# lesliegaga/GPT-SoVITS

Hardware: AMD Instinct MI355X
Metric: synthesised audio sec/sec (1/RTF), v2 pipeline (higher is better)
Workload: dtype f16

## Files before the change

gpt-sovits_amd/csrc/attn.hip:

```cpp
#include <stdlib.h>

#include "engine.h"

#define GSV_PIN() do { asm volatile("" ::: "memory"); __builtin_amdgcn_sched_barrier(0); } while (0)

namespace gsv {

__device__ __forceinline__ f4 mma16(h8 a, h8 b, f4 c) { return __builtin_amdgcn_mfma_f32_16x16x32_f16(a, b, c, 0, 0, 0); }

__global__ __launch_bounds__(256) void vt_kernel(const _Float16* __restrict__ v, int ld, int T, int ldv, _Float16* __restrict__ vt,
                                                 int heads, _Float16* __restrict__ q, int ldq, _Float16* __restrict__ k, int ldk,
                                                 const float* __restrict__ rope_cs, int rope_half, int planes, long long xz,
                                                 long long vtz) {
  const int row = blockIdx.z / planes, plane = blockIdx.z - row * planes;
  v += row * xz; q += row * xz; k += row * xz; vt += row * vtz;
  if (plane == heads) {
    const int n = T * rope_half * 2;
    const int stride = gridDim.x * gridDim.y * 256;
    for (int i = (blockIdx.y * gridDim.x + blockIdx.x) * 256 + threadIdx.x; i < n; i += stride) {
      const int which = i / (T * rope_half);
      const int rr = i - which * T * rope_half;
      const int t = rr / rope_half, p = rr - t * rope_half;
      _Float16* x = (which ? k + (long long)t * ldk : q + (long long)t * ldq) + 2 * p;
      const float c = rope_cs[((long long)t * rope_half + p) * 2], sn = rope_cs[((long long)t * rope_half + p) * 2 + 1];
// ... 142 lines not shown
}

template <int QT>
static int launch_flash_qt(const void* q, int ldq, const void* k, int ldk, const void* vt_buf, int ldv, int T, int heads, float scale,
                           void* out, int ldo, hipStream_t s, int rows, long long xz, long long vtz, long long oz) {
  const size_t lds = ((size_t)4 * 16 * QT * 68 + 8 * 16 * QT) * 4;
  static bool attr = false;
  if (!attr) {
    GSV_HIP(hipFuncSetAttribute((const void*)flash_attn64_f16_kernel<QT>, hipFuncAttributeMaxDynamicSharedMemorySize, (int)lds));
    attr = true;
  }
  hipLaunchKernelGGL(flash_attn64_f16_kernel<QT>, dim3(cdiv(T, 16 * QT), rows * heads), dim3(256), lds, s, (const _Float16*)q, ldq,
                     (const _Float16*)k, ldk, (const _Float16*)vt_buf, ldv, T, scale, (_Float16*)out, ldo, heads, xz, vtz, oz);
  GSV_HIP(hipGetLastError());
  return GSV_OK;
}

__device__ __forceinline__ int4 seg_find(const int4* __restrict__ tab, int n_seg, int x, bool by_tile) {
  int lo = 0, hi = n_seg - 1;
  while (lo < hi) {
    const int mid = (lo + hi + 1) >> 1;
    const int4 e = tab[mid];
    if ((by_tile ? e.w : e.z) <= x) lo = mid; else hi = mid - 1;
  }
  return tab[lo];
}

__global__ __launch_bounds__(256) void vt_seg_kernel(const _Float16* __restrict__ v, int ld, const int4* __restrict__ tab, int n_seg,
                                                     int ldv, _Float16* __restrict__ vt) {
  __shared__ _Float16 tile[32][34];
  const int head = blockIdx.z, j0 = blockIdx.x * 32, c0 = blockIdx.y * 32;
  const int4 sg = seg_find(tab, n_seg, j0, false);
  const int k0 = j0 - sg.z;
  const int tx = threadIdx.x & 31, ty = threadIdx.x >> 5;
  for (int i = ty; i < 32; i += 8) {
    const int j = k0 + i;
    tile[i][tx] = j < sg.y ? v[(long long)(sg.x + j) * ld + head * 64 + c0 + tx] : (_Float16)0.f;
  }
  __syncthreads();
  for (int i = ty; i < 32; i += 8) vt[((long long)head * 64 + c0 + i) * ldv + j0 + tx] = tile[tx][i];
}

template <int QT>
__global__ __launch_bounds__(256) void flash_attn64_seg_f16_kernel(const _Float16* __restrict__ q, int ldq, const _Float16* __restrict__ k,
                                                                   int ldk, const _Float16* __restrict__ vt, int ldv,
                                                                   const int4* __restrict__ tab, int n_seg, float scale,
                                                                   _Float16* __restrict__ out, int ldo) {
  const int vid = xcd_virtual_id(blockIdx.y * gridDim.x + blockIdx.x, gridDim.x * gridDim.y);
  const int head = vid / gridDim.x, tile = vid % gridDim.x;
  const int4 sg = seg_find(tab, n_seg, tile, true);
  flash_attn64_tile<QT>(q + (long long)sg.x * ldq, ldq, k + (long long)sg.x * ldk, ldk, vt + sg.z, ldv, sg.y, scale,
                        out + (long long)sg.x * ldo, ldo, head, (tile - sg.w) * (16 * QT));
}

template <int QT>
static int launch_flash_seg_qt(const void* q, int ldq, const void* k, int ldk, const void* vt_buf, int ldv, const int4* tab, int n_seg,
                               int tiles, int heads, float scale, void* out, int ldo, hipStream_t s) {
  const size_t lds = ((size_t)4 * 16 * QT * 68 + 8 * 16 * QT) * 4;
  static bool attr = false;
  if (!attr) {
    GSV_HIP(hipFuncSetAttribute((const void*)flash_attn64_seg_f16_kernel<QT>, hipFuncAttributeMaxDynamicSharedMemorySize, (int)lds));
    attr = true;
  }
  GSV_LAUNCH(flash_attn64_seg_f16_kernel<QT>, dim3(tiles, heads), dim3(256), lds, s, (const _Float16*)q, ldq, (const _Float16*)k, ldk,
             (const _Float16*)vt_buf, ldv, tab, n_seg, scale, (_Float16*)out, ldo);
  return GSV_OK;
}

__global__ __launch_bounds__(256) void vt96_kernel(const _Float16* __restrict__ v, int ld, int T, int ldv, _Float16* __restrict__ vt) {
  __shared__ _Float16 tile[32][34];
  const int head = blockIdx.z, j0 = blockIdx.x * 32, c0 = blockIdx.y * 32;
  const int tx = threadIdx.x & 31, ty = threadIdx.x >> 5;
  for (int i = ty; i < 32; i += 8) {
    const int j = j0 + i;
    tile[i][tx] = j < T ? v[(long long)j * ld + head * 96 + c0 + tx] : (_Float16)0.f;
  }
  __syncthreads();
  for (int i = ty; i < 32; i += 8) {
    const int j = j0 + tx;
    if (j < ldv) vt[((long long)head * 96 + c0 + i) * ldv + j] = tile[tx][i];
  }
}

template <int QT>
__global__ __launch_bounds__(256) void flash_rel96_f16_kernel(const _Float16* __restrict__ q, int ldq, const _Float16* __restrict__ k,
                                                              int ldk, const _Float16* __restrict__ vt, int ldv, int T, float scale,
                                                              const float* __restrict__ rel_k, const float* __restrict__ rel_v,
                                                              _Float16* __restrict__ out, int ldo, const int* __restrict__ kr) {
  constexpr int D = 96, KS = 3, DT = 6, W = 4, NB = 9, LDO = 100, BQ = 16 * QT;
  extern __shared__ float smem[];
  float* Os = smem;
  float* Ms = Os + 4 * BQ * LDO;
  float* Ls = Ms + 4 * BQ;
  float* Bias = Ls + 4 * BQ;
  float* Sb = Bias + BQ * NB;
  const int vid = xcd_virtual_id(blockIdx.y * gridDim.x + blockIdx.x, gridDim.x * gridDim.y);
  const int head = vid / gridDim.x, q0 = (vid % gridDim.x) * BQ;
  const int lane = threadIdx.x & 63, wave = threadIdx.x >> 6;
  const int r = lane & 15, g = lane >> 4;
  h8 qf[QT][KS];
#pragma unroll
  for (int t = 0; t < QT; ++t) {
    const _Float16* qp = q + (long long)min(q0 + 16 * t + r, T - 1) * ldq + head * D + g * 8;
#pragma unroll
    for (int ks = 0; ks < KS; ++ks) qf[t][ks] = *(const h8*)(qp + 32 * ks);
  }
  for (int i = threadIdx.x; i < BQ * NB; i += 256) Sb[i] = -INFINITY;
#pragma unroll
  for (int t = 0; t < QT; ++t) {
    if ((t & 3) != wave) continue;
#pragma unroll
    for (int rr = 0; rr < NB; ++rr) {
      float sdot = 0.f;
#pragma unroll
      for (int ks = 0; ks < KS; ++ks)
#pragma unroll
        for (int e = 0; e < 8; ++e) sdot += (float)qf[t][ks][e] * rel_k[rr * D + ks * 32 + g * 8 + e];
      sdot += __shfl_xor(sdot, 16, 64);
      sdot += __shfl_xor(sdot, 32, 64);
      if (g == 0) Bias[(16 * t + r) * NB + rr] = sdot * scale;
    }
  }
  __syncthreads();
  const _Float16* kh = k + head * D + g * 8;
  const _Float16* vh = vt + (long long)head * D * ldv + (long long)r * ldv + 8 * g;
  const int kra = 8 * (r >> 2) + (r & 3);
  f4 o[QT][DT];
  float m[QT], l[QT];
#pragma unroll
  for (int t = 0; t < QT; ++t) {
    m[t] = -INFINITY; l[t] = 0.f;
#pragma unroll
    for (int d = 0; d < DT; ++d) o[t][d] = (f4){0.f, 0.f, 0.f, 0.f};
  }
  int klo[QT], khi[QT];
#pragma unroll
  for (int t = 0; t < QT; ++t) {
    const int qi = min(q0 + 16 * t + r, T - 1);
    klo[t] = kr ? kr[2 * qi] : 0;
    khi[t] = kr ? kr[2 * qi + 1] : T;
  }
  const int c0 = kr ? kr[2 * q0] >> 5 : 0;
  const int nchunks = kr ? (kr[2 * min(q0 + BQ - 1, T - 1) + 1] + 31) >> 5 : (T + 31) >> 5, lastc = nchunks - 1;
  struct KV { h8 ka[KS], kb[KS]; h8 v[DT]; };
  auto fetch = [&](KV& f, int c) {
    const int key0 = c << 5;
    const _Float16* pa = kh + (long long)min(key0 + kra, T - 1) * ldk;
    const _Float16* pb = kh + (long long)min(key0 + kra + 4, T - 1) * ldk;
#pragma unroll
    for (int ks = 0; ks < KS; ++ks) { f.ka[ks] = *(const h8*)(pa + 32 * ks); f.kb[ks] = *(const h8*)(pb + 32 * ks); }
#pragma unroll
    for (int d = 0; d < DT; ++d) f.v[d] = *(const h8*)(vh + (long long)(d * 16) * ldv + key0);
  };
  auto process = [&](const KV& f, int c, bool valid) {
    const int key0 = c << 5;
#pragma unroll
    for (int t = 0; t < QT; ++t) {
      f4 sa = (f4){0.f, 0.f, 0.f, 0.f}, sb = sa;
#pragma unroll
      for (int ks = 0; ks < KS; ++ks) { sa = mma16(f.ka[ks], qf[t][ks], sa); sb = mma16(f.kb[ks], qf[t][ks], sb); }
      float p[8];
#pragma unroll
      for (int i = 0; i < 4; ++i) {
        const int ja = key0 + 8 * g + i, jb = ja + 4;
        p[i] = (valid && ja >= klo[t] && ja < khi[t]) ? sa[i] * scale : -INFINITY;
        p[4 + i] = (valid && jb >= klo[t] && jb < khi[t]) ? sb[i] * scale : -INFINITY;
      }
      const int qt0 = q0 + 16 * t;
      if (valid && key0 + 31 >= qt0 - W && key0 <= qt0 + 15 + W) {
        const int qi = qt0 + r;
#pragma unroll
        for (int i = 0; i < 8; ++i) {
          const int j = key0 + 8 * g + i;
          const int rp = j - qi + W;
          if (rp >= 0 && rp < NB && j >= klo[t] && j < khi[t] && qi < T) {
            p[i] += Bias[(16 * t + r) * NB + rp];
            Sb[(16 * t + r) * NB + rp] = p[i];
          }
        }
      }
      float mx = -INFINITY;
#pragma unroll
      for (int i = 0; i < 8; ++i) mx = fmaxf(mx, p[i]);
      mx = fmaxf(mx, __shfl_xor(mx, 16, 64));
      mx = fmaxf(mx, __shfl_xor(mx, 32, 64));
      const float mnew = fmaxf(m[t], mx), msafe = mnew == -INFINITY ? 0.f : mnew;
      const float alpha = __expf(m[t] - msafe);
      float ps = 0.f;
#pragma unroll
      for (int i = 0; i < 8; ++i) { p[i] = __expf(p[i] - msafe); ps += p[i]; }
      ps += __shfl_xor(ps, 16, 64);
      ps += __shfl_xor(ps, 32, 64);
      l[t] = l[t] * alpha + ps;
      m[t] = mnew;
      const h8 pf = (h8){(_Float16)p[0], (_Float16)p[1], (_Float16)p[2], (_Float16)p[3], (_Float16)p[4], (_Float16)p[5], (_Float16)p[6], (_Float16)p[7]};
#pragma unroll
      for (int d = 0; d < DT; ++d) {
        o[t][d] *= alpha;
        o[t][d] = mma16(f.v[d], pf, o[t][d]);
      }
    }
  };
  KV fA, fB;
  fetch(fA, min(c0 + wave, lastc));
  for (int c = c0 + wave; c < nchunks; c += 8) {
    fetch(fB, min(c + 4, lastc));
    GSV_PIN();
    process(fA, c, true);
    GSV_PIN();
    fetch(fA, min(c + 8, lastc));
    GSV_PIN();
    process(fB, c + 4, c + 4 < nchunks);
    GSV_PIN();
  }
#pragma unroll
  for (int t = 0; t < QT; ++t) {
#pragma unroll
    for (int d = 0; d < DT; ++d) *(f4*)&Os[((size_t)wave * BQ + 16 * t + r) * LDO + d * 16 + 4 * g] = o[t][d];
    if (g == 0) { Ms[wave * BQ + 16 * t + r] = m[t]; Ls[wave * BQ + 16 * t + r] = l[t]; }
  }
  __syncthreads();
  for (int it = threadIdx.x; it < BQ * (D / 4); it += 256) {
    const int qq = it / (D / 4), d4 = (it % (D / 4)) * 4;
    if (q0 + qq >= T) continue;
    const float mt = fmaxf(fmaxf(Ms[qq], Ms[BQ + qq]), fmaxf(Ms[2 * BQ + qq], Ms[3 * BQ + qq]));
    float den = 0.f;
    f4 acc = (f4){0.f, 0.f, 0.f, 0.f};
#pragma unroll
    for (int w = 0; w < 4; ++w) {
      const float e = __expf(Ms[w * BQ + qq] - mt);
      den += e * Ls[w * BQ + qq];
      acc += *(const f4*)&Os[((size_t)w * BQ + qq) * LDO + d4] * e;
    }
#pragma unroll
    for (int rr = 0; rr < NB; ++rr) {
      const float pw = __expf(Sb[qq * NB + rr] - mt);
      const f4 rv = *(const f4*)(rel_v + rr * D + d4);
      acc += rv * pw;
    }
    const float inv = 1.f / den;
    *(h4*)(out + (long long)(q0 + qq) * ldo + head * D + d4) =
        (h4){(_Float16)(acc[0] * inv), (_Float16)(acc[1] * inv), (_Float16)(acc[2] * inv), (_Float16)(acc[3] * inv)};
  }
}

int launch_flash_rel96_f16(const void* q, int ldq, const void* k, int ldk, const void* v, int ldvv, void* vt_buf, int T, int heads,
                           float scale, const float* rel_k, const float* rel_v, void* out, int ldo, hipStream_t s, const int* kr) {
  GSV_REQUIRE(T >= 1 && heads >= 1 && rel_k && rel_v, "flash_rel96: bad argument");
  GSV_REQUIRE(ldq % 8 == 0 && ldk % 8 == 0 && ldo % 4 == 0 && ((uintptr_t)q % 16) == 0 && ((uintptr_t)k % 16) == 0 && ((uintptr_t)out % 8) == 0 &&
              ((uintptr_t)rel_v % 16) == 0, "flash_rel96: operands must be 16-byte aligned with leading dims multiple of 8");
  const int ldv = (T + 31) / 32 * 32;
  hipLaunchKernelGGL(vt96_kernel, dim3(ldv / 32, 3, heads), dim3(256), 0, s, (const _Float16*)v, ldvv, T, ldv, (_Float16*)vt_buf);
  constexpr int QT = 2;
  set_attn_route(ATTN_REL96, QT);
  const size_t lds = ((size_t)4 * 16 * QT * 100 + 8 * 16 * QT + 2 * 16 * QT * 9) * 4;
  static bool attr = false;
  if (!attr) {
    GSV_HIP(hipFuncSetAttribute((const void*)flash_rel96_f16_kernel<QT>, hipFuncAttributeMaxDynamicSharedMemorySize, (int)lds));
    attr = true;
  }
  hipLaunchKernelGGL(flash_rel96_f16_kernel<QT>, dim3(cdiv(T, 16 * QT), heads), dim3(256), lds, s, (const _Float16*)q, ldq,
                     (const _Float16*)k, ldk, (const _Float16*)vt_buf, ldv, T, scale, rel_k, rel_v, (_Float16*)out, ldo, kr);
  GSV_HIP(hipGetLastError());
  return GSV_OK;
}

int launch_flash_attn64_f16_rows(const void* q, int ldq, const void* k, int ldk, const void* v, int ldvv, void* vt_buf, int T, int heads,
                                 float scale, void* out, int ldo, hipStream_t s, const float* rope_cs, int rope_half, int rows,
                                 long long xz, long long vtz, long long oz, int qt_arg) {
  GSV_REQUIRE(T >= 1 && heads >= 1 && rows >= 1, "flash_attn: empty problem");
  GSV_REQUIRE(qt_arg == 0 || qt_arg == 1 || qt_arg == 2 || qt_arg == 4, "flash_attn: qt %d is not 0 (by shape), 1, 2 or 4", qt_arg);
  GSV_REQUIRE(ldq % 8 == 0 && ldk % 8 == 0 && ldo % 4 == 0 && ((uintptr_t)q % 16) == 0 && ((uintptr_t)k % 16) == 0 && ((uintptr_t)out % 8) == 0,
              "flash_attn: operands must be 16-byte aligned with leading dims multiple of 8");
  const int ldv = (T + 31) / 32 * 32;
  const int planes = heads + (rope_cs ? 1 : 0);
  GSV_REQUIRE(rows == 1 || (xz % 8 == 0 && vtz % 8 == 0 && oz % 4 == 0 && vtz >= (long long)heads * 64 * ldv),
              "flash_attn: row strides must keep every row 16-byte aligned and its V^T buffer apart");
  GSV_REQUIRE((long long)rows * planes <= 65535 && (long long)rows * heads <= 65535, "flash_attn: %d rows x %d heads exceed the grid", rows, heads);
  hipLaunchKernelGGL(vt_kernel, dim3(ldv / 32, 2, rows * planes), dim3(256), 0, s, (const _Float16*)v, ldvv, T, ldv, (_Float16*)vt_buf, heads,
                     (_Float16*)const_cast<void*>(q), ldq, (_Float16*)const_cast<void*>(k), ldk, rope_cs, rope_half, planes, xz, vtz);
  static const int qt_env = getenv("GSV_FLASH_QT") ? atoi(getenv("GSV_FLASH_QT")) : 0;
  int qt = qt_arg ? qt_arg : qt_env ? qt_env : ((long long)cdiv(T, 64) * heads >= 200 ? 4 : ((long long)cdiv(T, 32) * heads >= 200 ? 2 : 1));
  set_attn_route(ATTN_ROWS, qt >= 4 ? 4 : qt >= 2 ? 2 : 1);
  if (qt >= 4) return launch_flash_qt<4>(q, ldq, k, ldk, vt_buf, ldv, T, heads, scale, out, ldo, s, rows, xz, vtz, oz);
  if (qt >= 2) return launch_flash_qt<2>(q, ldq, k, ldk, vt_buf, ldv, T, heads, scale, out, ldo, s, rows, xz, vtz, oz);
  return launch_flash_qt<1>(q, ldq, k, ldk, vt_buf, ldv, T, heads, scale, out, ldo, s, rows, xz, vtz, oz);
}

int launch_flash_attn64_f16(const void* q, int ldq, const void* k, int ldk, const void* v, int ldvv, void* vt_buf, int T, int heads,
                            float scale, void* out, int ldo, hipStream_t s, const float* rope_cs, int rope_half) {
  return launch_flash_attn64_f16_rows(q, ldq, k, ldk, v, ldvv, vt_buf, T, heads, scale, out, ldo, s, rope_cs, rope_half, 1, 0, 0, 0);
}

int launch_flash_attn64_f16_seg(const void* q, int ldq, const void* k, int ldk, const void* v, int ldvv, void* vt_buf, int n_seg,
                                const int* seg_lens, int heads, float scale, void* out, int ldo, hipStream_t s, int qt_arg) {
  GSV_REQUIRE(q && k && v && vt_buf && out && seg_lens, "flash_attn_seg: null argument");
  GSV_REQUIRE(qt_arg == 0 || qt_arg == 1 || qt_arg == 2 || qt_arg == 4, "flash_attn_seg: qt %d is not 0 (by shape), 1, 2 or 4", qt_arg);
  GSV_REQUIRE(n_seg >= 1 && heads >= 1 && heads <= 65535, "flash_attn_seg: %d segments, %d heads", n_seg, heads);
  GSV_REQUIRE(n_seg <= gsveng::kSegTableMax, "flash_attn_seg: %d segments exceed the table's %d", n_seg, gsveng::kSegTableMax);
  GSV_REQUIRE(ldq % 8 == 0 && ldk % 8 == 0 && ldo % 4 == 0 && ((uintptr_t)q % 16) == 0 && ((uintptr_t)k % 16) == 0 && ((uintptr_t)out % 8) == 0 &&
              ((uintptr_t)vt_buf % 16) == 0, "flash_attn_seg: operands must be 16-byte aligned with leading dims multiple of 8");
  long long rows = 0, t32 = 0, t64 = 0;
  for (int i = 0; i < n_seg; ++i) {
    GSV_REQUIRE(seg_lens[i] >= 1, "flash_attn_seg: segment %d has length %d", i, seg_lens[i]);
    rows += seg_lens[i]; t32 += cdiv(seg_lens[i], 32); t64 += cdiv(seg_lens[i], 64);
  }
  GSV_REQUIRE(rows + 32LL * n_seg <= 0x7fffffffLL, "flash_attn_seg: %lld rows exceed the index range", rows);
  static const int qt_env = getenv("GSV_FLASH_QT") ? atoi(getenv("GSV_FLASH_QT")) : 0;
  const int qt = qt_arg ? qt_arg : qt_env ? (qt_env >= 4 ? 4 : qt_env >= 2 ? 2 : 1) : (t64 * heads >= 200 ? 4 : (t32 * heads >= 200 ? 2 : 1));
  gsveng::SegTable tb;
  GSV_RC(gsveng::seg_table_begin(&tb));
  long long row0 = 0, col0 = 0, tile0 = 0;
  for (int i = 0; i < n_seg; ++i) {
    tb.image[4 * i] = (int)row0; tb.image[4 * i + 1] = seg_lens[i]; tb.image[4 * i + 2] = (int)col0; tb.image[4 * i + 3] = (int)tile0;
    row0 += seg_lens[i]; col0 += 32 * cdiv(seg_lens[i], 32); tile0 += cdiv(seg_lens[i], 16 * qt);
  }
  const int ldv = (int)col0, tiles = (int)tile0;
  GSV_REQUIRE(tile0 * heads <= 0x7fffffffLL, "flash_attn_seg: %lld query tiles x %d heads exceed the grid", tile0, heads);
  GSV_RC(gsveng::seg_table_upload(&tb, n_seg, s));
  const int4* tab = (const int4*)tb.dev;
  GSV_LAUNCH(vt_seg_kernel, dim3(ldv / 32, 2, heads), dim3(256), 0, s, (const _Float16*)v, ldvv, tab, n_seg, ldv, (_Float16*)vt_buf);
  set_attn_route(ATTN_SEG, qt);
  int rc;
  if (qt == 4) rc = launch_flash_seg_qt<4>(q, ldq, k, ldk, vt_buf, ldv, tab, n_seg, tiles, heads, scale, out, ldo, s);
  else if (qt == 2) rc = launch_flash_seg_qt<2>(q, ldq, k, ldk, vt_buf, ldv, tab, n_seg, tiles, heads, scale, out, ldo, s);
  else rc = launch_flash_seg_qt<1>(q, ldq, k, ldk, vt_buf, ldv, tab, n_seg, tiles, heads, scale, out, ldo, s);
  GSV_RC(rc);
  return gsveng::seg_table_end(&tb, s);
}

}
```

gpt-sovits_amd/csrc/vits.hip:

```cpp
#include "engine.h"

namespace gsv {

template <typename T>
__global__ void gather_rows_kernel(const int* __restrict__ idx, const float* __restrict__ table, int C, int rep, int n,
                                   T* __restrict__ out) {
  const int row = blockIdx.x;
  if (row >= n * rep) return;
  const float* src = table + (long long)idx[row / rep] * C;
  T* dst = out + (long long)row * C;
  for (int c = threadIdx.x; c < C; c += blockDim.x) dst[c] = (T)src[c];
}

template <typename T>
__global__ void gather_seg_kernel(const int* __restrict__ ids, const int* __restrict__ src, const float* __restrict__ table, int C,
                                  int rows, T* __restrict__ out) {
  const int row = blockIdx.x;
  if (row >= rows) return;
  const int i = src[row];
  T* dst = out + (long long)row * C;
  if (i < 0) { for (int c = threadIdx.x; c < C; c += blockDim.x) dst[c] = (T)0.f; return; }
  const float* sp = table + (long long)ids[i] * C;
  for (int c = threadIdx.x; c < C; c += blockDim.x) dst[c] = (T)sp[c];
}
// ... 112 lines not shown
  const int i0 = min((int)src, Tin - 1);
  const int i1 = min(i0 + 1, Tin - 1);
  const float w1 = src - (float)i0, w0 = 1.f - w1;
  for (int c = threadIdx.x; c < C; c += blockDim.x)
    dst[c] = (T)(w0 * to_f(xs[(long long)i0 * C + c]) + w1 * to_f(xs[(long long)i1 * C + c]));
}

template <typename T>
__global__ void interp_nearest_kernel(const T* __restrict__ x, int Tin, int Tout, int C, float scale, T* __restrict__ y) {
  const int t = blockIdx.x;
  const int src = min((int)floorf((float)t * scale), Tin - 1);
  for (int c = threadIdx.x; c < C; c += blockDim.x) y[(long long)t * C + c] = x[(long long)src * C + c];
}

__global__ void sv_prelu_acc_kernel(const float* __restrict__ ge_ref, const float* __restrict__ sv_proj, const float* __restrict__ a,
                                    float wgt, int accumulate, int n, float* __restrict__ ge) {
  int i = blockIdx.x * blockDim.x + threadIdx.x;
  if (i >= n) return;
  const float v = ge_ref[i] + sv_proj[i];
  const float u = (v >= 0.f ? v : a[i] * v) * wgt;
  ge[i] = accumulate ? ge[i] + u : u;
}

__global__ void vec_add_kernel(const float* a, const float* b, float* out, int n) {
  int i = blockIdx.x * blockDim.x + threadIdx.x;
  if (i < n) out[i] = a[i] + b[i];
}

__global__ void argmax_code_kernel(const float* __restrict__ dots, const float* __restrict__ x, const float* __restrict__ ee,
                                   int D, int NB, int* __restrict__ codes) {
  const int t = blockIdx.x, lane = threadIdx.x;
  float xx = 0.f;
  for (int c = lane; c < D; c += 64) { float v = x[(long long)t * D + c]; xx += v * v; }
  xx = wave_sum(xx);
  float best = -INFINITY; int bi = 0x7fffffff;
  for (int j = lane; j < NB; j += 64) {
    float d = -(xx - 2.f * dots[(long long)t * NB + j] + ee[j]);
    if (d > best) { best = d; bi = j; }
  }
  for (int o = 32; o > 0; o >>= 1) {
    float ov = __shfl_xor(best, o, 64); int oi = __shfl_xor(bi, o, 64);
    if (ov > best || (ov == best && oi < bi)) { best = ov; bi = oi; }
  }
  if (lane == 0) codes[t] = bi;
}

}

using namespace gsv;


struct AttnLayerW { Conv qkv, o; float *rel_k = nullptr, *rel_v = nullptr; float *g1 = nullptr, *b1 = nullptr, *g2 = nullptr, *b2 = nullptr; Conv f1, f2; };
struct WNW { std::vector<Conv> in, res; std::vector<float*> in_bias_eff; Conv cond; };
struct FlowW { Conv pre, post; WNW wn; };

struct gsv_vits : gsveng::Ctx {
  gsv_vits() : Ctx("vits") {}
  gsv_vits_config cfg;
  bool has_ref = false;
  Conv ssl_proj_enc, proj, c_pre, text_pre, c_post, mq, mkv, mo;
  std::vector<AttnLayerW> enc_ssl, enc_text, enc2;
  float *text_emb = nullptr, *codebook = nullptr, *code_ee = nullptr;
  Conv top_ssl_proj;
  void* codebook_t = nullptr;
  FlowW flows[4];
  Conv conv_pre, conv_post, cond;
  float* conv_pre_bias_eff = nullptr;
  GenW gen;
  Conv bridge, w1_pre, w1_proj;
  WNW w1;
  Conv sv_emb, ge_to512;
  float *prelu_w = nullptr, *ge_ref = nullptr, *sv_proj = nullptr, *ge512 = nullptr;
  void* sv_t = nullptr;
  Conv r_sp0, r_sp3, r_t0, r_t1, r_qkv, r_fc, r_out;
  float* ge = nullptr;
  void* ge_t = nullptr;
  float* mo_bias_eff = nullptr;
  float* voices = nullptr;
  int voice_len = 0, voice_off_pre = 0, voice_off_in = 0;
  std::vector<char> voice_ok;
  gsveng::SegUpload seg;
  hipStream_t ref_stream = nullptr;
  gsveng::GenTap dbg_last;
  int lastF = 0;
  hipEvent_t ev[4] = {nullptr, nullptr, nullptr, nullptr};
  float last_total_ms = 0.f, last_gen_ms = 0.f;
};

using namespace gsveng;

namespace gsveng {

int make_encoder(gsv_vits* h, const std::string& prefix, int n_layers, std::vector<AttnLayerW>* out) {
  const auto& c = h->cfg;
  const int H = c.hidden_channels, FC = c.filter_channels, kc = H / c.n_heads;
  out->resize(n_layers);
  for (int i = 0; i < n_layers; ++i) {
    AttnLayerW& L = (*out)[i];
    const std::string a = prefix + ".attn_layers." + std::to_string(i) + ".";
    GSV_RC(make_stacked(h, {a + "conv_q", a + "conv_k", a + "conv_v"}, H, H, &L.qkv));
    GSV_RC(make_conv(h, a + "conv_o", H, H, 1, true, &L.o));
    GSV_RC(make_vec(h, a + "emb_rel_k", (size_t)9 * kc, &L.rel_k));
    GSV_RC(make_vec(h, a + "emb_rel_v", (size_t)9 * kc, &L.rel_v));
    GSV_RC(make_vec(h, prefix + ".norm_layers_1." + std::to_string(i) + ".gamma", H, &L.g1));
    GSV_RC(make_vec(h, prefix + ".norm_layers_1." + std::to_string(i) + ".beta", H, &L.b1));
    GSV_RC(make_vec(h, prefix + ".norm_layers_2." + std::to_string(i) + ".gamma", H, &L.g2));
    GSV_RC(make_vec(h, prefix + ".norm_layers_2." + std::to_string(i) + ".beta", H, &L.b2));
    const std::string f = prefix + ".ffn_layers." + std::to_string(i) + ".";
    GSV_RC(make_conv(h, f + "conv_1", FC, H, c.kernel_size, true, &L.f1));
    GSV_RC(make_conv(h, f + "conv_2", H, FC, c.kernel_size, true, &L.f2));
  }
  return GSV_OK;
}

static int make_wn(gsv_vits* h, const std::string& prefix, int NL, int H, int GIN, WNW* w) {
  w->in.resize(NL); w->res.resize(NL); w->in_bias_eff.resize(NL);
  for (int li = 0; li < NL; ++li) {
    GSV_RC(make_conv(h, prefix + ".in_layers." + std::to_string(li), 2 * H, H, 5, true, &w->in[li]));
    GSV_RC(make_conv(h, prefix + ".res_skip_layers." + std::to_string(li), li < NL - 1 ? 2 * H : H, H, 1, true, &w->res[li]));
    GSV_RC(dalloc(h, (void**)&w->in_bias_eff[li], (size_t)2 * H * 4));
  }
  return make_conv(h, prefix + ".cond_layer", 2 * H * NL, GIN, 1, true, &w->cond);
}

int run_encoder(gsv_vits* h, hipStream_t s, std::vector<AttnLayerW>& layers, void* x, int Tn, const int* row_seg = nullptr,
                const int* kr = nullptr) {
  const auto& c = h->cfg;
  const int H = c.hidden_channels, FC = c.filter_channels, kc = H / c.n_heads;
  const size_t es = esz(h);
  void *qkv, *ao, *y, *ff;
  GSV_RC(need(h, "enc_qkv", (size_t)Tn * 3 * H * es, &qkv));
  GSV_RC(need(h, "enc_ao", (size_t)Tn * H * es, &ao));
  GSV_RC(need(h, "enc_y", (size_t)Tn * H * es, &y));
  GSV_RC(need(h, "enc_ff", (size_t)Tn * FC * es, &ff));
  for (auto& L : layers) {
    ConvOpt o;
    GSV_RC(conv(h, s, L.qkv, x, H, Tn, qkv, Tn, o));
    GSV_RC(attention(h, s, qkv, 3 * H, 0, qkv, 3 * H, H, 2 * H, Tn, Tn, c.n_heads, kc, 1.f / sqrtf((float)kc), L.rel_k, L.rel_v, ao, H, kr));
    GSV_RC(conv(h, s, L.o, ao, H, Tn, y, Tn, o));
    GSV_RC(launch_layernorm(h->dtype, x, 0, y, 0, L.g1, L.b1, x, 0, Tn, H, 1e-5f, s, row_seg));
    ConvOpt o1; o1.post_act = ACT_RELU; o1.row_seg = row_seg;
    GSV_RC(conv(h, s, L.f1, x, H, Tn, ff, Tn, o1));
    GSV_RC(conv(h, s, L.f2, ff, FC, Tn, y, Tn, o));
    GSV_RC(launch_layernorm(h->dtype, x, 0, y, 0, L.g2, L.b2, x, 0, Tn, H, 1e-5f, s, row_seg));
  }
  return GSV_OK;
}

int seg_gap(const gsv_vits_config& c) {
  int g = 1;
  g = std::max(g, conv_reach(c.kernel_size, 1));
  g = std::max(g, conv_reach(5, 1));
  GenW shape;
  gen_shape(c, &shape);
  return std::max(g, gen_gap(shape));
}

struct SegLayout {
  int n = 0, G = 0, F = 0, L = 0, Fn = 0;
  std::vector<int> f0, l0, c0, p0, fn0, nf;
};

int seg_layout(const gsv_vits_config& c, int n, const int* code_lens, const int* phone_lens, const double* speeds, SegLayout* o) {
  GSV_REQUIRE(n >= 1 && n <= 4096 && code_lens && phone_lens, "vits segments: bad segment count %d", n);
  o->n = n; o->G = seg_gap(c);
  o->f0.resize(n); o->l0.resize(n); o->c0.resize(n); o->p0.resize(n); o->fn0.resize(n); o->nf.resize(n);
// ... 279 lines not shown
    GSV_RC(dalloc(h, (void**)&h->sv_proj, (size_t)GIN * 4));
    GSV_RC(dalloc(h, (void**)&h->ge512, (size_t)MH * 4));
    GSV_RC(dalloc(h, &h->sv_t, (size_t)20480 * esz(h)));
  }
  for (auto& e : h->ev) GSV_HIP(hipEventCreate(&e));
  h->staged.clear();
  h->finalized = true;
  return GSV_OK;
}

int gsv_vits_set_refer(gsv_vits_t* h, const float* const* specs, const int* frames, int bins, int n_refs, gsv_stream_t stream) {
  GSV_REQUIRE(h && h->finalized, "vits_set_refer: handle not finalized");
  GSV_REQUIRE(!h->cfg.v2pro, "vits_set_refer: a v2Pro model needs gsv_vits_set_refer_sv (one sv embedding per reference)");
  return GSV_WITH_T(h, set_refer_impl<T>(h, specs, frames, bins, nullptr, n_refs, stream));
}

int gsv_vits_set_refer_sv(gsv_vits_t* h, const float* const* specs, const int* frames, int bins, const float* const* sv_embs,
                          int n_refs, gsv_stream_t stream) {
  GSV_REQUIRE(h && h->finalized, "vits_set_refer_sv: handle not finalized");
  GSV_REQUIRE(h->cfg.v2pro && sv_embs, "vits_set_refer_sv: not a v2Pro model, or no sv embeddings");
  for (int r = 0; r < n_refs; ++r) GSV_REQUIRE(sv_embs[r], "vits_set_refer_sv: missing sv embedding %d", r);
  return GSV_WITH_T(h, set_refer_impl<T>(h, specs, frames, bins, sv_embs, n_refs, stream));
}

}

namespace gsveng {
template <typename T>
static int run_wn(gsv_vits* h, hipStream_t s, const WNW& w, int F, void* hb, void* xin, void* acts, void* wout, const SegRun* sr,
                  size_t voff, int Lm) {
  const int NL = (int)w.in.size(), H = w.in[0].cin;
  const int* seg_f = sr ? sr->seg_p : nullptr;
  for (int li = 0; li < NL; ++li) {
    GSV_RC(conv_voice(h, s, w.in[li], hb, F, xin, ConvOpt(), w.in_bias_eff[li], sr, voff + (size_t)li * 2 * H, seg_f));
    GSV_LAUNCH(gate_kernel<T>, dim3(nblk((long long)F * H)), dim3(256), 0, s, (const T*)xin, (long long)F * H, H, (T*)acts);
    if (li < NL - 1) {
      ConvOpt ores; ores.cout = H; ores.w_row0 = 0; ores.accumulate = 1; ores.row_seg = seg_f;
      GSV_RC(conv(h, s, w.res[li], acts, H, F, hb, F, ores));
      if (Lm < F) GSV_HIP(hipMemsetAsync((T*)hb + (size_t)Lm * H, 0, (size_t)(F - Lm) * H * sizeof(T), s));
      ConvOpt osk; osk.cout = H; osk.w_row0 = H; osk.accumulate = li > 0;
      GSV_RC(conv(h, s, w.res[li], acts, H, F, wout, F, osk));
    } else {
      ConvOpt osk; osk.accumulate = li > 0;
      GSV_RC(conv(h, s, w.res[li], acts, H, F, wout, F, osk));
    }
  }
  return GSV_OK;
}

template <typename T>
static int decode_wav(gsv_vits* h, hipStream_t s, const int32_t* codes, int Tc, const int32_t* phones, int L, double speed,
                      const float* noise, float noise_scale, uint64_t seed, float* wav, const SegRun* sr) {
  const auto& c = h->cfg;
  void* y = nullptr;
  int F = 0;
  GSV_RC(run_enc_p<T>(h, s, codes, Tc, phones, L, speed, &y, &F, sr));
  const size_t es = sizeof(T);
  const int H = c.hidden_channels, IC = c.inter_channels;
  const int* seg_f = sr ? sr->seg_p : nullptr;
  float* stats;
  GSV_RC(need(h, "stats", (size_t)F * 2 * IC * 4, (void**)&stats));
  { ConvOpt of; of.out_f32 = 1; GSV_RC(conv(h, s, h->proj, y, H, F, stats, F, of)); }
  void *z, *zf, *hb, *xin, *acts, *wout;
  GSV_RC(need(h, "z", (size_t)F * IC * es, &z));
  GSV_RC(need(h, "zf", (size_t)F * IC * es, &zf));
  GSV_RC(need(h, "wn_h", (size_t)F * H * es, &hb));
  GSV_RC(need(h, "wn_xin", (size_t)F * 2 * H * es, &xin));
  GSV_RC(need(h, "wn_acts", (size_t)F * H * es, &acts));
  GSV_RC(need(h, "wn_out", (size_t)F * H * es, &wout));
  GSV_LAUNCH(zp_kernel<T>, dim3(nblk((long long)F * IC)), dim3(256), 0, s, stats, F, IC, noise, noise_scale, (unsigned long long)seed, (T*)z,
             seg_f, sr ? sr->start : nullptr, sr ? sr->noff : nullptr, sr ? sr->seeds : nullptr, sr ? sr->post->Fn : 0);
  const int half = IC / 2;
  for (int fi = 3; fi >= 0; --fi) {
    FlowW& f = h->flows[fi];
    GSV_LAUNCH(flip_channels_kernel<T>, dim3(nblk((long long)F * IC)), dim3(256), 0, s, (const T*)z, (long long)F * IC, IC, (T*)zf);
    std::swap(z, zf);
    ConvOpt om; om.row_seg = seg_f;
    GSV_RC(conv(h, s, f.pre, z, IC, F, hb, F, om));
    GSV_RC(run_wn<T>(h, s, f.wn, F, hb, xin, acts, wout, sr, h->voice_off_in + (size_t)fi * 4 * 2 * H, F));
    ConvOpt op; op.scale = -1.f; op.accumulate = 1; op.ldy = IC; op.y_col0 = half; op.row_seg = seg_f;
    GSV_RC(conv(h, s, f.post, wout, H, F, z, F, op));
  }
  h->lastF = F;
  {
    void* zkeep;
    GSV_RC(need(h, "z_keep", (size_t)F * IC * es, &zkeep));
    GSV_HIP(hipMemcpyAsync(zkeep, z, (size_t)F * IC * es, hipMemcpyDeviceToDevice, s));
  }
  GSV_HIP(hipEventRecord(h->ev[1], s));
  void* gb[5];
  GSV_RC(gen_buffers(h, h->gen, "g", F, gb));
  void* cur = gb[3];
  GSV_RC(conv_voice(h, s, h->conv_pre, z, F, cur, ConvOpt(), h->conv_pre_bias_eff, sr, h->voice_off_pre, seg_f));
  int Tn = F;
  GSV_RC(run_generator_stages(h, s, h->gen, gb, &cur, &Tn, seg_f ? sr->seg_up.data() : nullptr, nullptr, &h->dbg_last));
  float* wout_p = wav;
  if (seg_f) GSV_RC(need(h, "wav_pad", (size_t)Tn * 4, (void**)&wout_p));
  { ConvOpt op; op.pre_act = ACT_LRELU; op.pre_slope = 0.01f; op.post_act = ACT_TANH; op.out_f32 = 1;
    GSV_RC(conv(h, s, h->conv_post, cur, h->conv_post.cin, Tn, wout_p, Tn, op)); }
  if (seg_f) {
    const int up = Tn / F;
    GSV_RC(launch_compact_wav(s, wout_p, seg_f, up, (long long)sr->post->G * up, (long long)Tn, wav));
  }
  GSV_HIP(hipEventRecord(h->ev[2], s));
  return GSV_OK;
}

template <typename T>
static int decode_encp(gsv_vits* h, hipStream_t s, const int32_t* codes, int Tc, const int32_t* phones, int L, double speed, float* fea) {
  const auto& c = h->cfg;
  const size_t es = sizeof(T);
  const int H = c.hidden_channels, W = 512;
  void* y = nullptr;
  int Fs = 0;
  GSV_RC(run_enc_p<T>(h, s, codes, Tc, phones, L, speed, &y, &Fs));
  const double sf = c.flavor == 1 ? 1.875 : 2.0;
  const int F = (int)floor((double)Fs * sf);
  const double per = c.flavor == 1 ? 3.875 : 4.0;
  const int sizee = (speed == 1.0) ? (int)((double)Tc * per) : (int)((double)Tc * per / speed) + 1;
  const int Lm = std::min(sizee, F);
  void *br, *up, *hb, *xin, *acts, *wout, *st;
  GSV_RC(need(h, "e_br", (size_t)Fs * W * es, &br));
  GSV_RC(need(h, "e_up", (size_t)F * W * es, &up));
  GSV_RC(need(h, "e_h", (size_t)F * W * es, &hb));
  GSV_RC(need(h, "e_xin", (size_t)F * 2 * W * es, &xin));
  GSV_RC(need(h, "e_acts", (size_t)F * W * es, &acts));
  GSV_RC(need(h, "e_out", (size_t)F * W * es, &wout));
  GSV_RC(need(h, "e_st", (size_t)F * W * es, &st));
  auto mask_tail = [&](void* p) -> int {
    if (Lm < F) GSV_HIP(hipMemsetAsync((char*)p + (size_t)Lm * W * es, 0, (size_t)(F - Lm) * W * es, s));
    return GSV_OK;
  };
  { ConvOpt ob; ob.post_act = ACT_LRELU01; GSV_RC(conv(h, s, h->bridge, y, H, Fs, br, Fs, ob)); }
  GSV_LAUNCH(interp_nearest_kernel<T>, dim3(F), dim3(128), 0, s, (const T*)br, Fs, F, W, (float)(1.0 / sf), (T*)up);
  ConvOpt o;
  GSV_RC(conv(h, s, h->w1_pre, up, W, F, hb, F, o));
  GSV_RC(mask_tail(hb));
  GSV_RC(run_wn<T>(h, s, h->w1, F, hb, xin, acts, wout, nullptr, 0, Lm));
  GSV_RC(mask_tail(wout));
  GSV_RC(conv(h, s, h->w1_proj, wout, W, F, st, F, o));
  GSV_RC(mask_tail(st));
  GSV_LAUNCH(cl_to_cf_kernel<T>, dim3(nblk((long long)F * W)), dim3(256), 0, s, (const T*)st, F, W, 0, W, fea);
  return GSV_OK;
}

template <typename T>
static int extract_latent(gsv_vits* h, hipStream_t s, const float* ssl, int T50, int32_t* codes) {
  const auto& c = h->cfg;
  const int SSL = c.ssl_dim, T25 = (T50 - 2) / 2 + 1;
  void* x; float *p, *dots;
  GSV_RC(need(h, "xl_x", (size_t)T50 * SSL * sizeof(T), &x));
  GSV_RC(need(h, "xl_p", (size_t)T25 * SSL * 4, (void**)&p));
  GSV_RC(need(h, "xl_d", (size_t)T25 * c.n_bins * 4, (void**)&dots));
  GSV_RC(cf_to_cl(h, s, ssl, T50, SSL, x));
  ConvOpt o; o.stride = 2; o.pad = 0; o.out_f32 = 1;
  GSV_RC(conv(h, s, h->top_ssl_proj, x, SSL, T50, p, T25, o));
  void* pt;
  GSV_RC(need(h, "xl_pt", (size_t)T25 * SSL * sizeof(T), &pt));
  GSV_RC(launch_convert(p, pt, h->dtype, (long long)T25 * SSL, s));
  ConvArgs a;
  a.x = pt; a.w = h->codebook_t; a.y = dots; a.out_f32 = 1;
  a.T_in = T25; a.T_out = T25; a.T_virt = T25; a.Cin = SSL; a.Cout = c.n_bins; a.ldx = SSL; a.ldw = SSL; a.ldy = c.n_bins;
  GSV_RC(launch_conv_gemm(h->dtype, a, s));
  GSV_LAUNCH(argmax_code_kernel, dim3(T25), dim3(64), 0, s, dots, p, h->code_ee, SSL, c.n_bins, codes);
  return GSV_OK;
}

template <typename T>
static int debug_cl_to_cf(hipStream_t s, const void* src, int Tn, int C, float* out) {
  GSV_LAUNCH(cl_to_cf_kernel<T>, dim3(nblk((long long)Tn * C)), dim3(256), 0, s, (const T*)src, Tn, C, 0, C, out);
  return GSV_OK;
// ... 138 lines not shown
  sr.lay = &lay; sr.post = interp ? &post : &lay;
  sr.seg_f = dm + o_sf; sr.seg_l = dm + o_sl; sr.kr_f = dm + o_kf; sr.kr_l = dm + o_kl; sr.kr_x = dm + o_kx;
  sr.src_code = dm + o_sc; sr.src_phone = dm + o_sp; sr.start = dm + o_st; sr.noff = dm + o_no; sr.seeds = dseed; sr.bias = vb;
  sr.seg_p = interp ? dm + o_pf : sr.seg_f;
  if (interp) { sr.start_pre = dm + o_ps; sr.len_pre = dm + o_pi; sr.len_post = dm + o_po; }
  if (n == 1) {
    sr.seg_f = sr.seg_l = sr.seg_p = sr.kr_f = sr.kr_l = sr.kr_x = nullptr;
  }
  long long up = 1;
  for (int i = 0; i < h->cfg.n_ups && n > 1; ++i) {
    up *= h->cfg.up_rates[i];
    const std::string nm = "seg_up" + std::to_string(i);
    int* su;
    GSV_RC(need(h, nm.c_str(), (size_t)Fp * up * 4, (void**)&su));
    GSV_RC(launch_expand_seg(s, sr.seg_p, (int)up, (long long)Fp * up, su));
    sr.seg_up.push_back(su);
  }
  GSV_HIP(hipEventRecord(h->ev[0], s));
  return GSV_WITH_T(h, decode_wav<T>(h, s, codes, 0, phones, L, 1.0, noise, noise_scale, seeds[0], wav, &sr));
}

int gsv_vits_encp_frames(gsv_vits_t* h, int T, double speed) {
  if (!h || T < 1 || !(speed > 0.0)) return -1;
  const int F0 = 2 * T;
  const int Fs = (speed == 1.0) ? F0 : (int)((double)F0 / speed) + 1;
  const double sf = h->cfg.flavor == 1 ? 1.875 : 2.0;
  return (int)floor((double)Fs * sf);
}

int gsv_vits_decode_encp(gsv_vits_t* h, const int32_t* codes, int Tc, const int32_t* phones, int L, double speed, float* fea,
                         gsv_stream_t stream) {
  GSV_REQUIRE(h && h->finalized, "vits_decode_encp: handle not finalized");
  GSV_REQUIRE(h->cfg.flavor != 0, "vits_decode_encp: this handle is a v1/v2 model (use gsv_vits_decode)");
  GSV_REQUIRE(h->has_ref, "vits_decode_encp: call gsv_vits_set_refer first");
  GSV_REQUIRE(codes && phones && fea && Tc >= 1 && L >= 1, "vits_decode_encp: empty input (T=%d, L=%d)", Tc, L);
  GSV_REQUIRE(speed > 0.0, "vits_decode_encp: speed must be positive");
  return GSV_WITH_T(h, decode_encp<T>(h, (hipStream_t)stream, codes, Tc, phones, L, speed, fea));
}

int gsv_vits_last_timing(gsv_vits_t* h, float* total_ms, float* generator_ms) {
  GSV_REQUIRE(h && h->finalized && h->lastF > 0, "vits_last_timing: no decode yet");
  GSV_HIP(hipEventSynchronize(h->ev[2]));
  float a = 0.f, b = 0.f;
  GSV_HIP(hipEventElapsedTime(&a, h->ev[0], h->ev[2]));
  GSV_HIP(hipEventElapsedTime(&b, h->ev[1], h->ev[2]));
  if (total_ms) *total_ms = a;
  if (generator_ms) *generator_ms = b;
  return GSV_OK;
}

int gsv_vits_extract_latent(gsv_vits_t* h, const float* ssl, int T50, int32_t* codes, gsv_stream_t stream) {
  GSV_REQUIRE(h && h->finalized && ssl && codes, "vits_extract_latent: bad argument");
  GSV_REQUIRE(T50 >= 2, "vits_extract_latent: need at least 2 ssl frames (got %d)", T50);
  return GSV_WITH_T(h, extract_latent<T>(h, (hipStream_t)stream, ssl, T50, codes));
}

int gsv_vits_debug_tensor(gsv_vits_t* h, const char* name, float* out, int64_t cap, int64_t* numel, gsv_stream_t stream) {
  GSV_REQUIRE(h && h->finalized && name && out && numel, "vits_debug_tensor: bad argument");
  hipStream_t s = (hipStream_t)stream;
  const auto& c = h->cfg;
  const std::string n(name);
  const int F = h->lastF, IC = c.inter_channels;
  if (n == "ge") {
    GSV_REQUIRE(cap >= c.gin_channels, "vits_debug_tensor: buffer too small");
    GSV_HIP(hipMemcpyAsync(out, h->ge, (size_t)c.gin_channels * 4, hipMemcpyDeviceToDevice, s));
    *numel = c.gin_channels;
    return GSV_OK;
  }
  GSV_REQUIRE(F > 0, "vits_debug_tensor: no decode yet");
  if (n == "gen_last_in") {
    const GenTap& tap = h->dbg_last;
    const long long ne = (long long)tap.T * tap.C;
    GSV_REQUIRE(tap.in && cap >= ne, "vits_debug_tensor: buffer too small");
    *numel = ne;
    return GSV_WITH_T(h, debug_cl_to_cf<T>(s, tap.in, tap.T, tap.C, out));
  }
  GSV_REQUIRE(cap >= (int64_t)F * IC, "vits_debug_tensor: buffer too small");
  *numel = (int64_t)F * IC;
  if (n == "m_p" || n == "logs_p") {
    const float* st = (const float*)h->bufs["stats"].p;
    GSV_LAUNCH(cl_to_cf_kernel<float>, dim3(nblk((long long)F * IC)), dim3(256), 0, s, st, F, 2 * IC, n == "m_p" ? 0 : IC, IC, out);
    return GSV_OK;
  }
  if (n == "z") return GSV_WITH_T(h, debug_cl_to_cf<T>(s, h->bufs["z_keep"].p, F, IC, out));
  set_error("vits_debug_tensor: unknown tensor '%s' (ge, m_p, logs_p, z, gen_last_in)", name);
  return GSV_ERR_ARG;
}

}
```

Before: 2917.

## Streamline rel96 flash attention and drop debug z copy from decode path

In the rel96 flash attention kernel, chunks that are fully in range skip per-key masking. The row max and sum reductions use permlane16/32 swaps instead of shuffles, and the output rescale is skipped when alpha is 1 across the whole wavefront. The launcher can pick a QT=4 tile variant for large unmasked problems, with an environment override. Separately, the VITS decode no longer copies z into a debug buffer each call and keeps a pointer instead, which risks the debug tensor being overwritten by later work.

```diff
diff --git a/gpt-sovits_amd/csrc/attn.hip b/gpt-sovits_amd/csrc/attn.hip
--- a/gpt-sovits_amd/csrc/attn.hip
+++ b/gpt-sovits_amd/csrc/attn.hip
@@ -248,6 +248,15 @@
   }
 }
 
+template <bool MAX>
+__device__ __forceinline__ float quad_reduce(float x) {
+  auto op = [](unsigned a, unsigned b) { return MAX ? fmaxf(__uint_as_float(a), __uint_as_float(b)) : __uint_as_float(a) + __uint_as_float(b); };
+  const auto rows = __builtin_amdgcn_permlane16_swap(__float_as_uint(x), __float_as_uint(x), false, false);
+  x = op(rows[0], rows[1]);
+  const auto halves = __builtin_amdgcn_permlane32_swap(__float_as_uint(x), __float_as_uint(x), false, false);
+  return op(halves[0], halves[1]);
+}
+
 template <int QT>
 __global__ __launch_bounds__(256) void flash_rel96_f16_kernel(const _Float16* __restrict__ q, int ldq, const _Float16* __restrict__ k,
                                                               int ldk, const _Float16* __restrict__ vt, int ldv, int T, float scale,
@@ -326,11 +335,16 @@
 #pragma unroll
       for (int ks = 0; ks < KS; ++ks) { sa = mma16(f.ka[ks], qf[t][ks], sa); sb = mma16(f.kb[ks], qf[t][ks], sb); }
       float p[8];
-#pragma unroll
-      for (int i = 0; i < 4; ++i) {
-        const int ja = key0 + 8 * g + i, jb = ja + 4;
-        p[i] = (valid && ja >= klo[t] && ja < khi[t]) ? sa[i] * scale : -INFINITY;
-        p[4 + i] = (valid && jb >= klo[t] && jb < khi[t]) ? sb[i] * scale : -INFINITY;
+      if (!kr && valid && key0 + 32 <= T) {
+#pragma unroll
+        for (int i = 0; i < 4; ++i) { p[i] = sa[i] * scale; p[4 + i] = sb[i] * scale; }
+      } else {
+#pragma unroll
+        for (int i = 0; i < 4; ++i) {
+          const int ja = key0 + 8 * g + i, jb = ja + 4;
+          p[i] = (valid && ja >= klo[t] && ja < khi[t]) ? sa[i] * scale : -INFINITY;
+          p[4 + i] = (valid && jb >= klo[t] && jb < khi[t]) ? sb[i] * scale : -INFINITY;
+        }
       }
       const int qt0 = q0 + 16 * t;
       if (valid && key0 + 31 >= qt0 - W && key0 <= qt0 + 15 + W) {
@@ -348,23 +362,22 @@
       float mx = -INFINITY;
 #pragma unroll
       for (int i = 0; i < 8; ++i) mx = fmaxf(mx, p[i]);
-      mx = fmaxf(mx, __shfl_xor(mx, 16, 64));
-      mx = fmaxf(mx, __shfl_xor(mx, 32, 64));
+      mx = quad_reduce<true>(mx);
       const float mnew = fmaxf(m[t], mx), msafe = mnew == -INFINITY ? 0.f : mnew;
       const float alpha = __expf(m[t] - msafe);
       float ps = 0.f;
 #pragma unroll
       for (int i = 0; i < 8; ++i) { p[i] = __expf(p[i] - msafe); ps += p[i]; }
-      ps += __shfl_xor(ps, 16, 64);
-      ps += __shfl_xor(ps, 32, 64);
+      ps = quad_reduce<false>(ps);
       l[t] = l[t] * alpha + ps;
       m[t] = mnew;
       const h8 pf = (h8){(_Float16)p[0], (_Float16)p[1], (_Float16)p[2], (_Float16)p[3], (_Float16)p[4], (_Float16)p[5], (_Float16)p[6], (_Float16)p[7]};
-#pragma unroll
-      for (int d = 0; d < DT; ++d) {
-        o[t][d] *= alpha;
-        o[t][d] = mma16(f.v[d], pf, o[t][d]);
+      if (__any(alpha != 1.f)) {
+#pragma unroll
+        for (int d = 0; d < DT; ++d) o[t][d] *= alpha;
       }
+#pragma unroll
+      for (int d = 0; d < DT; ++d) o[t][d] = mma16(f.v[d], pf, o[t][d]);
     }
   };
   KV fA, fB;
@@ -410,14 +423,9 @@
   }
 }
 
-int launch_flash_rel96_f16(const void* q, int ldq, const void* k, int ldk, const void* v, int ldvv, void* vt_buf, int T, int heads,
-                           float scale, const float* rel_k, const float* rel_v, void* out, int ldo, hipStream_t s, const int* kr) {
-  GSV_REQUIRE(T >= 1 && heads >= 1 && rel_k && rel_v, "flash_rel96: bad argument");
-  GSV_REQUIRE(ldq % 8 == 0 && ldk % 8 == 0 && ldo % 4 == 0 && ((uintptr_t)q % 16) == 0 && ((uintptr_t)k % 16) == 0 && ((uintptr_t)out % 8) == 0 &&
-              ((uintptr_t)rel_v % 16) == 0, "flash_rel96: operands must be 16-byte aligned with leading dims multiple of 8");
-  const int ldv = (T + 31) / 32 * 32;
-  hipLaunchKernelGGL(vt96_kernel, dim3(ldv / 32, 3, heads), dim3(256), 0, s, (const _Float16*)v, ldvv, T, ldv, (_Float16*)vt_buf);
-  constexpr int QT = 2;
+template <int QT>
+static int launch_flash_rel96_qt(const void* q, int ldq, const void* k, int ldk, const void* vt_buf, int ldv, int T, int heads, float scale,
+                                 const float* rel_k, const float* rel_v, void* out, int ldo, hipStream_t s, const int* kr) {
   set_attn_route(ATTN_REL96, QT);
   const size_t lds = ((size_t)4 * 16 * QT * 100 + 8 * 16 * QT + 2 * 16 * QT * 9) * 4;
   static bool attr = false;
@@ -429,6 +437,20 @@
                      (const _Float16*)k, ldk, (const _Float16*)vt_buf, ldv, T, scale, rel_k, rel_v, (_Float16*)out, ldo, kr);
   GSV_HIP(hipGetLastError());
   return GSV_OK;
+}
+
+int launch_flash_rel96_f16(const void* q, int ldq, const void* k, int ldk, const void* v, int ldvv, void* vt_buf, int T, int heads,
+                           float scale, const float* rel_k, const float* rel_v, void* out, int ldo, hipStream_t s, const int* kr) {
+  GSV_REQUIRE(T >= 1 && heads >= 1 && rel_k && rel_v, "flash_rel96: bad argument");
+  GSV_REQUIRE(ldq % 8 == 0 && ldk % 8 == 0 && ldo % 4 == 0 && ((uintptr_t)q % 16) == 0 && ((uintptr_t)k % 16) == 0 && ((uintptr_t)out % 8) == 0 &&
+              ((uintptr_t)rel_v % 16) == 0, "flash_rel96: operands must be 16-byte aligned with leading dims multiple of 8");
+  static const int forced_qt = [] { const char* e = getenv("GSV_REL96_QT"); return e ? atoi(e) : 0; }();
+  GSV_REQUIRE(forced_qt == 0 || forced_qt == 2 || forced_qt == 4, "flash_rel96: GSV_REL96_QT must be 2 or 4");
+  const int ldv = (T + 31) / 32 * 32;
+  hipLaunchKernelGGL(vt96_kernel, dim3(ldv / 32, 3, heads), dim3(256), 0, s, (const _Float16*)v, ldvv, T, ldv, (_Float16*)vt_buf);
+  const bool wide = forced_qt ? forced_qt == 4 : !kr && (long long)cdiv(T, 32) * heads > 256;
+  return wide ? launch_flash_rel96_qt<4>(q, ldq, k, ldk, vt_buf, ldv, T, heads, scale, rel_k, rel_v, out, ldo, s, kr)
+              : launch_flash_rel96_qt<2>(q, ldq, k, ldk, vt_buf, ldv, T, heads, scale, rel_k, rel_v, out, ldo, s, kr);
 }
 
 int launch_flash_attn64_f16_rows(const void* q, int ldq, const void* k, int ldk, const void* v, int ldvv, void* vt_buf, int T, int heads,
diff --git a/gpt-sovits_amd/csrc/vits.hip b/gpt-sovits_amd/csrc/vits.hip
--- a/gpt-sovits_amd/csrc/vits.hip
+++ b/gpt-sovits_amd/csrc/vits.hip
@@ -218,6 +218,7 @@
   gsveng::SegUpload seg;
   hipStream_t ref_stream = nullptr;
   gsveng::GenTap dbg_last;
+  const void* dbg_z = nullptr;
   int lastF = 0;
   hipEvent_t ev[4] = {nullptr, nullptr, nullptr, nullptr};
   float last_total_ms = 0.f, last_gen_ms = 0.f;
@@ -663,11 +664,7 @@
     GSV_RC(conv(h, s, f.post, wout, H, F, z, F, op));
   }
   h->lastF = F;
-  {
-    void* zkeep;
-    GSV_RC(need(h, "z_keep", (size_t)F * IC * es, &zkeep));
-    GSV_HIP(hipMemcpyAsync(zkeep, z, (size_t)F * IC * es, hipMemcpyDeviceToDevice, s));
-  }
+  h->dbg_z = z;
   GSV_HIP(hipEventRecord(h->ev[1], s));
   void* gb[5];
   GSV_RC(gen_buffers(h, h->gen, "g", F, gb));
@@ -972,7 +969,10 @@
     GSV_LAUNCH(cl_to_cf_kernel<float>, dim3(nblk((long long)F * IC)), dim3(256), 0, s, st, F, 2 * IC, n == "m_p" ? 0 : IC, IC, out);
     return GSV_OK;
   }
-  if (n == "z") return GSV_WITH_T(h, debug_cl_to_cf<T>(s, h->bufs["z_keep"].p, F, IC, out));
+  if (n == "z") {
+    GSV_REQUIRE(h->dbg_z, "vits_debug_tensor: no waveform decode yet");
+    return GSV_WITH_T(h, debug_cl_to_cf<T>(s, h->dbg_z, F, IC, out));
+  }
   set_error("vits_debug_tensor: unknown tensor '%s' (ge, m_p, logs_p, z, gen_last_in)", name);
   return GSV_ERR_ARG;
 }
```

Measured after the change: 2953 (median of 3 runs). No clear change (+1.2%).
